# tum-vision/tandem

Measured on AMD Instinct MI355X. Metric: depth-maps/sec @ 640×480×7-view×3-stage; TSDF voxels integrated/sec, higher is better.
Workload: dtype f32; 1 GPU; 640x480 ref+6-src keyframe window, 3-stage cascade (48/32/8 hypotheses), view aggregation, fp32; independent windows, 4 in flight per GPU (one DrMvsnet engine each) x 1 GPU replica(s); trained weights recovered from the reference's exported tandem_512x320 model (same architecture), inputs resident in HBM; height=480, width=640, views=7, parallelism=replicas x1, 4 engines per GPU

## Files before the change

tandem_amd/csrc/dr_mvsnet.hip:

```cpp
#include <atomic>
#include <memory>

#include <dlfcn.h>
#include <rccl/rccl.h>

#include "conv_mfma.h"
#include "mvs_host.h"
#include "mvs_launch.h"
#ifdef DR_PARITY_HOOKS
#include "tail_kernels.h"
#endif
#include "fn_front.h"
#include "fn_head3.h"

namespace dr {

std::string &last_error_slot() {
  thread_local std::string s;
  return s;
}

struct DevTensor {
  float *d = nullptr;
  int D = 0, H = 0, W = 0, C = 0;
  int pad = 0;
  int split = 0;
  size_t n() const { return (size_t)D * (H + 2 * pad) * (W + 2 * pad) * C; }
  float *interior() const { return d + ((size_t)pad * (W + 2 * pad) + pad) * C; }
};

struct Op {
  enum Kind { PREPROCESS, CONV, SKIPUP, PROB, COSTVOL, REGRESS, EDGE, HIST, SCAN, APPLY, BORDERFIX, TAIL, FRONT, HEAD3 } kind;
  const float *p0 = nullptr, *p1 = nullptr, *p3 = nullptr, *p4 = nullptr;
  float *p2 = nullptr;
  int d0 = 0, d1 = 0, d2 = 0;
  std::string name;
  ConvLaunch conv;
#ifdef DR_PARITY_HOOKS
  TailArgs tail{};
#endif
  FrontArgs front{};
  Head3Args head3{};
  PreprocessArgs pre{};
  std::function<ConvLaunch(int)> replan;
  std::string sig;
  int ncand = 0;
  int stage = 0, shift = 0, bits = 0;
  double flops = 0, bytes = 0;
};

struct Rccl {
  void *lib = nullptr;
  decltype(&ncclGetUniqueId) GetUniqueId = nullptr;
  decltype(&ncclCommInitRank) CommInitRank = nullptr;
  decltype(&ncclCommDestroy) CommDestroy = nullptr;
  decltype(&ncclAllReduce) AllReduce = nullptr;
  decltype(&ncclReduce) Reduce = nullptr;
  decltype(&ncclBroadcast) Broadcast = nullptr;
  decltype(&ncclGetErrorString) GetErrorString = nullptr;
  decltype(&ncclCommCount) CommCount = nullptr;
  static Rccl &get() {
    static Rccl r;
    static std::mutex m;
    std::lock_guard<std::mutex> g(m);
    if (!r.lib) {
      if (const char *e = getenv("DR_RCCL_LIB")) r.lib = dlopen(e, RTLD_NOW | RTLD_GLOBAL);
      else
      for (const char *n : {"librccl.so.1", "librccl.so", "/opt/rocm/lib/librccl.so.1"})
        if ((r.lib = dlopen(n, RTLD_NOW | RTLD_GLOBAL))) break;
      if (!r.lib) fail(DR_ERR_UNSUPPORTED, "RCCL not found (librccl.so.1): %s", dlerror());
      r.GetUniqueId = reinterpret_cast<decltype(r.GetUniqueId)>(dlsym(r.lib, "ncclGetUniqueId"));
      r.CommInitRank = reinterpret_cast<decltype(r.CommInitRank)>(dlsym(r.lib, "ncclCommInitRank"));
      r.CommDestroy = reinterpret_cast<decltype(r.CommDestroy)>(dlsym(r.lib, "ncclCommDestroy"));
      r.AllReduce = reinterpret_cast<decltype(r.AllReduce)>(dlsym(r.lib, "ncclAllReduce"));
      r.Reduce = reinterpret_cast<decltype(r.Reduce)>(dlsym(r.lib, "ncclReduce"));
      r.Broadcast = reinterpret_cast<decltype(r.Broadcast)>(dlsym(r.lib, "ncclBroadcast"));
      r.GetErrorString = reinterpret_cast<decltype(r.GetErrorString)>(dlsym(r.lib, "ncclGetErrorString"));
      r.CommCount = reinterpret_cast<decltype(r.CommCount)>(dlsym(r.lib, "ncclCommCount"));
      if (!r.GetUniqueId || !r.CommInitRank || !r.CommDestroy || !r.AllReduce || !r.Reduce || !r.Broadcast || !r.GetErrorString) {
        r.lib = nullptr;
        fail(DR_ERR_UNSUPPORTED, "RCCL: missing symbols in librccl");
      }
    }
    return r;
  }
  void check(ncclResult_t e, const char *what) const {
    if (e != ncclSuccess) fail(DR_ERR_DEVICE, "RCCL %s: %s", what, GetErrorString(e));
  }
};

static const char *conv_kind_name(const ConvLaunch &c) {
  return c.async == 2 ? (c.march.rm ? "rowmarch" : (c.march.wino ? "winomarch" : "march")) : (c.async == 4 ? "wino" : (c.async ? "async" : ""));
}

class MvsEngine {
// ... 240 lines not shown
    DR_HIP(hipSetDevice(device_));
    const DevTensor &t = T(name);
    const size_t logical = (size_t)t.D * t.H * t.W * t.C;
    if (n) *n = logical;
    if (dims) { dims[0] = t.D; dims[1] = t.H; dims[2] = t.W; dims[3] = t.C; }
    if (out) {
      if (logical > n_max) fail(DR_ERR_ARG, "get_tensor(%s): need %zu floats, have %zu", name, logical, n_max);
      DR_HIP(hipStreamSynchronize(stream_));
      check_march();
      if (t.split) {
        const size_t npos = (size_t)t.D * t.H * t.W;
        for (int k = 0; k < t.C / t.split; ++k)
          DR_HIP(hipMemcpy2D(out + (size_t)k * t.split, (size_t)t.C * 4, t.d + (size_t)k * npos * t.split, (size_t)t.split * 4, (size_t)t.split * 4, npos, hipMemcpyDeviceToHost));
      } else if (!t.pad) DR_HIP(hipMemcpy(out, t.d, logical * 4, hipMemcpyDeviceToHost));
      else
        for (int z = 0; z < t.D; ++z)
          DR_HIP(hipMemcpy2D(out + (size_t)z * t.H * t.W * t.C, (size_t)t.W * t.C * 4, t.interior() + (size_t)z * (t.H + 2 * t.pad) * (t.W + 2 * t.pad) * t.C,
                             (size_t)(t.W + 2 * t.pad) * t.C * 4, (size_t)t.W * t.C * 4, t.H, hipMemcpyDeviceToHost));
    }
  }
  void profile(std::string &names, std::vector<float> &ms) {
    std::unique_lock<std::mutex> lk(mu_);
    require_config();
    if (comm_ && shard_nsrc_) fail(DR_ERR_PROTOCOL, "profile(): a view-sharded engine enqueues collectives -- every rank would have to profile in lockstep");
    DR_HIP(hipSetDevice(device_));
    forward(nullptr);
    std::vector<hipEvent_t> ev(ops_.size() + 1);
    for (auto &e : ev) DR_HIP(hipEventCreate(&e));
    forward(&ev);
    DR_HIP(hipStreamSynchronize(stream_));
    check_march();
    names.clear(); ms.clear();
    for (size_t i = 0; i < ops_.size(); ++i) {
      float t = 0;
      DR_HIP(hipEventElapsedTime(&t, ev[i], ev[i + 1]));
      ms.push_back(t);
      const Op &o = ops_[i];
      char kn[64] = "misc";
      if (o.kind == Op::CONV && o.conv.async == 2) snprintf(kn, sizeof kn, "k_conv_m<%d,%d,%d,%d,%d,%d,%d>", o.conv.ci, o.conv.nup, o.conv.ct, o.conv.pt, o.conv.fz, o.conv.ncw, o.conv.march.wino);
      else if (o.kind == Op::CONV && o.conv.async == 4) snprintf(kn, sizeof kn, "k_conv_w<%d,%d,%d>", o.conv.ci, o.conv.ct, o.conv.pt);
      else if (o.kind == Op::CONV && o.conv.async) snprintf(kn, sizeof kn, "k_conv_a<%d,%d,%d>", o.conv.ci, o.conv.ct, o.conv.pt);
      else if (o.kind == Op::CONV && o.conv.bf3) snprintf(kn, sizeof kn, "k_conv_b<%d,%d,%d>", o.conv.ci, o.conv.ct, o.conv.pt);
      else if (o.kind == Op::CONV && o.conv.args.class_loop > 0) snprintf(kn, sizeof kn, "k_conv_c<%d,%d,%d>", o.conv.ci, o.conv.ct, o.conv.pt);
      else if (o.kind == Op::CONV) snprintf(kn, sizeof kn, "k_conv<%d,%d,%d,%d>", o.conv.ci, o.conv.ct, o.conv.pt, o.conv.fz);
      else if (o.kind == Op::COSTVOL) choose_costvol(costvol_shape(cv_[o.stage - 1]), sw_, o.stage).name(kn, sizeof kn);
      else if (o.kind == Op::PROB) choose_prob(prob_shape(pr_[o.stage - 1]), sw_, o.stage).name(kn, sizeof kn);
#ifdef DR_PARITY_HOOKS
      else if (o.kind == Op::TAIL) snprintf(kn, sizeof kn, o.tail.wmf ? "k_tail_m<%d>" : "k_tail<%d>", std::max(3, tail_nout(o.tail.QY, o.tail.QX)));
#endif
      else if (o.kind == Op::REGRESS) snprintf(kn, sizeof kn, "k_regress");
      else if (o.kind == Op::PREPROCESS) snprintf(kn, sizeof kn, "k_preprocess");
      else if (o.kind == Op::FRONT) snprintf(kn, sizeof kn, "k_fn_front");
      else if (o.kind == Op::HEAD3) snprintf(kn, sizeof kn, "k_fn_head3");
      else if (o.kind == Op::SKIPUP) snprintf(kn, sizeof kn, "k_skip_up<%d>", o.stage);
      else if (o.kind == Op::BORDERFIX) snprintf(kn, sizeof kn, "k_out3_border");
      else snprintf(kn, sizeof kn, "k_filter");
      char line[256];
      snprintf(line, sizeof line, "%s\t%s\t%.6e\t%.6e\n", o.name.c_str(), kn, o.flops, o.bytes);
      names += line;
    }
    for (auto &e : ev) (void)hipEventDestroy(e);
  }
  void work(double *flops, double *bytes) {
    std::unique_lock<std::mutex> lk(mu_);
    require_config();
    double f = 0, b = 0;
    for (auto &o : ops_) { f += o.flops; b += o.bytes; }
    if (flops) *flops = f;
    if (bytes) *bytes = b;
  }

 private:
  void check_args(int H, int W, int V, int ref, const uint8_t *const *bgrs, const float *K9, const float *const *c2ws) {
    if (!bgrs || !K9 || !c2ws) fail(DR_ERR_ARG, "CallAsync: null pointer argument");
    const int vmin = shard_nsrc_ ? 1 : 2;
    if (V < vmin || V > kMaxSrc + 1) fail(DR_ERR_ARG, "CallAsync: view_num=%d unsupported (%d..%d)", V, vmin, kMaxSrc + 1);
    if (ref < 0 || ref >= V) fail(DR_ERR_ARG, "CallAsync: ref_index=%d out of range", ref);
    if (H <= 0 || W <= 0 || H % 32 || W % 32) fail(DR_ERR_ARG, "CallAsync: height/width must be positive multiples of 32 (got %dx%d)", H, W);
    for (int i = 0; i < V - 1; ++i) for (int j = i + 1; j < V; ++j)
      if (bgrs[i] == bgrs[j] || c2ws[i] == c2ws[j])
        fail(DR_ERR_ARG, "ERROR: In Call Async passing the same data for index %d and %d", i, j);
  }
  void require_config() { if (!H_) fail(DR_ERR_PROTOCOL, "no window uploaded yet"); }
  void rethrow_worker_error() {
    if (!worker_error_.empty()) { std::string e = worker_error_; worker_error_.clear(); fail(DR_ERR_DEVICE, "%s", e.c_str()); }
  }
  const float *take_result(std::unique_lock<std::mutex> &lk) {
    done_cv_.wait(lk, [&] { return !unprocessed_; });
    rethrow_worker_error();
    if (!has_output_) fail(DR_ERR_PROTOCOL, "Output should be valid. Maybe you called GetResult more than once?");
    has_output_ = false;
    return h_out_[out_cur_];
  }
  static std::atomic<int> &windows_in_flight(int device) {
    static std::atomic<int> n[16];
    return n[device & 15];
  }
  struct InFlight {
    int dev;
    InFlight(int d, bool counted_already) : dev(d) { if (!counted_already) windows_in_flight(dev).fetch_add(1, std::memory_order_relaxed); }
    ~InFlight() { windows_in_flight(dev).fetch_sub(1, std::memory_order_relaxed); }
  };
  void loop() {
    std::unique_lock<std::mutex> lk(mu_);
    while (running_) {
      if (unprocessed_) {
// ... 112 lines not shown
      if (P.launches.size() == 1) {
        o.replan = replan; o.ncand = ncand;
        char sig[160];
        snprintf(sig, sizeof sig, "%d, %d, %d, %d, %d, %d, %d, %d, %d, %d, %d, %d, %d", L.Cin, L.Cout, k3d, kh, kw, L.sd, L.sh, L.sw, L.transposed ? 1 : (L.up2 ? 1 + L.up2 : 0),
                 (int)mode + (fused ? 8 : 0) + (iS ? 16 : 0), iD, iH, iW);
        o.sig = sig;
      }
      o.flops = cl.flops;
      if (idx == 0) o.bytes = 4.0 * ((fused ? in.n() / in.C * fzc.cin + in.n() / 4 : in.n()) + out.n() + add_n);
      if (fused) o.flops += 2.0 * fzc.cin * in.C * (in.n() / in.C);
      ops_.push_back(o);
      ++idx;
    }
  }
  bool lds_fits(size_t bytes) const {
    int optin = 0;
    if (hipDeviceGetAttribute(&optin, hipDeviceAttributeSharedMemPerBlockOptin, device_) != hipSuccess || optin <= 0) {
      (void)hipGetLastError();
      if (hipDeviceGetAttribute(&optin, hipDeviceAttributeMaxSharedMemoryPerBlock, device_) != hipSuccess) { (void)hipGetLastError(); return false; }
    }
    return (size_t)optin >= bytes;
  }
  DevTensor &front_block(const std::string &fn, int V, int H, int W) {
    const HostTensor &wa = blob_.at(fn + "conv0.0.conv.weight"), &wb = blob_.at(fn + "conv0.1.conv.weight");
    const bool shape_ok = wa.dims.size() == 4 && wa.dims[0] == 8 && wa.dims[1] == 3 && wa.dims[2] == 3 && wa.dims[3] == 3 &&
                          wb.dims.size() == 4 && wb.dims[0] == 8 && wb.dims[1] == 8 && wb.dims[2] == 3 && wb.dims[3] == 3;
    const bool fits32 = (double)V * H * W * 32.0 < 2147483648.0 && ((uintptr_t)d_bgr_ & 3) == 0;
    if (!sw_.fn_front || conv_bf3_policy() || !shape_ok || !fits32 || !lds_fits(kFrontLdsBytes)) {
      DevTensor &img = alloc("image", V, H, W, 4);
      { Op o; o.kind = Op::PREPROCESS; o.name = "preprocess"; o.bytes = (double)V * H * W * (3 + 16); o.pre = {d_bgr_, reinterpret_cast<float4 *>(img.d), lut_, (size_t)V * H * W}; ops_.push_back(o); }
      DevTensor &c3a = cbr2("fn.conv0.0", fn + "conv0.0", img, 3, 1, CONV_XPAIR);
      return cbr2("fn.conv0.1", fn + "conv0.1", c3a, 3, 1, CONV_XPAIR);
    }
    DevTensor &c3 = alloc("fn.conv0.1", V, H, W, 8);
    Op o; o.kind = Op::FRONT; o.name = "fn.front";
    FrontArgs &a = o.front;
    a.bgr = d_bgr_; a.lut = lut_; a.out = c3.d;
    a.w1 = reinterpret_cast<const float4 *>(plan_arena_->upload(front_pack(wa.data.data(), 3, 4)));
    a.w2 = reinterpret_cast<const float4 *>(plan_arena_->upload(front_pack(wb.data.data(), 8, 8)));
    auto affine = [&](const std::string &bn) {
      std::vector<float> sc, bi, sb(32);
      fold_bn(blob_, bn, 8, sc, bi);
      for (int r = 0; r < 16; ++r) { sb[r] = sc[r & 7]; sb[16 + r] = bi[r & 7]; }
      return plan_arena_->upload(sb);
    };
    a.sb1 = affine(fn + "conv0.0.bn"); a.sb2 = affine(fn + "conv0.1.bn");
    a.V = V; a.H = H; a.W = W;
    a.tilesY = cdiv(H, kFrontTY); a.tilesX = cdiv(W, kFrontTXP); a.ntiles = V * a.tilesY * a.tilesX;
    o.flops = 2.0 * V * H * W * 9.0 * (4 * 8 + 8 * 8);
    o.bytes = (double)V * H * W * (3 + 32);
    ops_.push_back(o);
    return c3;
  }
  DevTensor &cbr2(const std::string &name, const std::string &p, const DevTensor &in, int k, int s, ConvMode m) {
    return add_conv(name, p + ".conv", p + ".bn", false, true, in, name, 1, k, k, 1, s, s, false, m, nullptr, 0);
  }
  DevTensor &cbr3(const std::string &name, const std::string &p, const DevTensor &in, int sd, int shw, ConvMode m) {
    return add_conv(name, p + ".conv", p + ".bn", false, true, in, name, 3, 3, 3, sd, shw, shw, false, m, nullptr, 0);
  }
  DevTensor &dbr3(const std::string &name, const std::string &p, const DevTensor &in, int sd, const DevTensor &skip) {
    return add_conv(name, p + ".conv", p + ".bn", false, true, in, name, 3, 3, 3, sd, 2, 2, true, CONV_NORMAL, &skip, 1);
  }

  void configure(int H, int W, int V) {
    if (H == H_ && W == W_ && V == V_) return;
    DR_HIP(hipStreamSynchronize(stream_));
    release();
    H_ = W_ = V_ = 0;
    memset(cv_, 0, sizeof cv_);
    memset(rg_, 0, sizeof rg_);
    memset(pr_, 0, sizeof pr_);
    try {
      build_plan(H, W, V);
    } catch (...) {
      release();
      throw;
    }
    H_ = H; W_ = W; V_ = V;
  }
  void build_featurenet(int V, int H, int W) {
    const std::string fn = "feature_net.";
    DevTensor &c3 = front_block(fn, V, H, W);
    DevTensor &c2a = cbr2("fn.conv1.0", fn + "conv1.0", c3, 5, 2, CONV_NORMAL);
    DevTensor &c2b = cbr2("fn.conv1.1", fn + "conv1.1", c2a, 3, 1, CONV_NORMAL);
    DevTensor &c2 = cbr2("fn.conv1.2", fn + "conv1.2", c2b, 3, 1, CONV_NORMAL);
    DevTensor &c1a = cbr2("fn.conv2.0", fn + "conv2.0", c2, 5, 2, CONV_NORMAL);
    DevTensor &c1b = cbr2("fn.conv2.1", fn + "conv2.1", c1a, 3, 1, CONV_NORMAL);
    DevTensor &c1 = cbr2("fn.conv2.2", fn + "conv2.2", c1b, 3, 1, CONV_NORMAL);
    const int fpad = sw_.costvol_v1 ? 0 : 1;
    add_conv("fn.out1", fn + "out.stage1", "", false, false, c1, "feat1", 1, 1, 1, 1, 1, 1, false, CONV_NORMAL, nullptr, 0, nullptr, fpad);
    fork_lo_ = ops_.size();
    DevTensor &i2 = add_skip("fn.skip2", fn + "skip.stage2", c2, "inter2", c1);
    add_conv("fn.out2", fn + "out.stage2", "", false, false, i2, "feat2", 1, 3, 3, 1, 1, 1, false, CONV_NORMAL, nullptr, 0, nullptr, fpad);
    feat2_op_ = ops_.size() - 1;
    const HostTensor &w3 = blob_.at(fn + "skip.stage3.weight");
    const HostTensor &wo3 = blob_.at(fn + "out.stage3.weight");
    if (sw_.out3_folded && !sw_.no_skip_fusion && !sw_.skip_on_conv && w3.dims[0] == 32 && w3.dims[1] == 8 && c3.C == 8 &&
        i2.C == 32 && wo3.dims[0] == 8 && wo3.dims[1] == 32 && i2.H * 2 == c3.H && i2.W * 2 == c3.W) {
      const Out3Fold fold = compose_out3(wo3.data, w3.data, blob_.at(fn + "skip.stage3.bias").data);
      const std::vector<float> &wa = fold.wa, &T = fold.T, &bint = fold.bint;
      DevTensor &f3 = alloc("feat3", c3.D, c3.H, c3.W, 8, fpad);
      if (sw_.fn_head3 && !conv_bf3_policy() && (double)f3.n() * 4.0 < 2147483648.0 && (double)i2.n() * 4.0 < 2147483648.0 && lds_fits(kH3LdsBytes)) {
        Op o; o.kind = Op::HEAD3; o.name = "fn.head3";
        Head3Args &a = o.head3;
        a.c0 = c3.d; a.i2 = i2.d;
        a.wa = reinterpret_cast<const float4 *>(plan_arena_->upload(h3_pack_a(wa.data())));
        a.wb = reinterpret_cast<const float4 *>(plan_arena_->upload(h3_pack_b(wo3.data.data())));
        std::vector<float> b16(16);
        for (int r = 0; r < 16; ++r) b16[r] = bint[r & 7];
        a.bias16 = plan_arena_->upload(b16); a.T = plan_arena_->upload(T);
        a.out = f3.interior(); a.V = c3.D; a.H = c3.H; a.W = c3.W;
        a.out_row = (f3.W + 2 * f3.pad) * 8; a.out_plane = (f3.H + 2 * f3.pad) * a.out_row;
        a.tilesY = cdiv(c3.H, kH3TY); a.tilesX = cdiv(c3.W, kH3TXP); a.ntiles = c3.D * a.tilesY * a.tilesX;
        o.flops = 2.0 * c3.D * c3.H * c3.W * (9.0 * 8 * 8 + 4.0 * 32 * 8);
        o.bytes = 4.0 * (c3.n() + i2.n() + (double)c3.D * c3.H * c3.W * 8);
        ops_.push_back(o);
      } else {
      ConvLayer LA; LA.Cin = 8; LA.Cout = 8; LA.kd = 1; LA.kh = 3; LA.kw = 3; LA.weight = wa.data(); LA.bias = bint; LA.out_pad = fpad;
      emit_conv("fn.out3a", LA, CONV_XPAIR, c3, f3, nullptr, 0, 0);
      for (int py = 0; py < 2; ++py) {
        ConvLayer LB; LB.Cin = 32; LB.Cout = 8; LB.kd = 1; LB.kh = 3; LB.kw = 3; LB.weight = wo3.data.data(); LB.up2 = 1 + py; LB.out_pad = fpad;
        emit_conv(py ? "fn.out3c" : "fn.out3b", LB, CONV_NORMAL, i2, f3, f3.interior(), 1, f3.n() / 2);
      }
      Op o; o.kind = Op::BORDERFIX; o.name = "fn.out3d"; o.p2 = f3.interior(); o.p1 = plan_arena_->upload(T); o.d0 = c3.D; o.d1 = c3.H; o.d2 = c3.W;
      o.stage = fpad; o.bytes = 64.0 * c3.D * (c3.H + c3.W);
      ops_.push_back(o);
      }
    } else
    if (!sw_.no_skip_fusion && !sw_.skip_on_conv && kParityHooks && w3.dims[0] == 32 && w3.dims[1] == 8 && c3.C == 8 && i2.C == 32 &&
        i2.H * 2 == c3.H && i2.W * 2 == c3.W) {
      ConvFuse fz{c3.d, plan_arena_->upload(w3.data), plan_arena_->upload(blob_.at(fn + "skip.stage3.bias").data), i2.d, 8};
      DevTensor virt; virt.D = c3.D; virt.H = c3.H; virt.W = c3.W; virt.C = 32; virt.d = nullptr;
      add_conv("fn.out3", fn + "out.stage3", "", false, false, virt, "feat3", 1, 3, 3, 1, 1, 1, false, CONV_XPAIR, nullptr, 0, &fz, fpad);
    } else {
      DevTensor &i3 = add_skip("fn.skip3", fn + "skip.stage3", c3, "inter3", i2);
      add_conv("fn.out3", fn + "out.stage3", "", false, false, i3, "feat3", 1, 3, 3, 1, 1, 1, false, CONV_XPAIR, nullptr, 0, nullptr, fpad);
    }
    fork_hi_ = ops_.size();
  }

  struct FnOut { size_t op; int stage; size_t offset; };
  struct FcBuffers { float *feat[3] = {nullptr, nullptr, nullptr}; uint8_t *bgr = nullptr; };
  static bool same_instance(const ConvLaunch &a, const ConvLaunch &b) {
    return a.async == b.async && a.ci == b.ci && a.ct == b.ct && a.pt == b.pt && a.fz == b.fz && a.bf3 == b.bf3 && a.nup == b.nup && a.ncw == b.ncw &&
           a.march.wino == b.march.wino && a.march.rm == b.march.rm;
  }
  void build_fn1(int H, int W) {
    fn1_ok_ = false; ops1_.clear(); fcache_.clear(); fc_.clear();
    if (ops_.empty() || ops_[0].kind != Op::FRONT || sw_.costvol_v1 || shard_nsrc_) return;
    const size_t lo = fork_lo_, hi = fork_hi_, f2 = feat2_op_;
    std::vector<Op> batch;
    batch.swap(ops_);
    tprefix_ = "c1.";
    try { build_featurenet(1, H, W); } catch (...) { tprefix_.clear(); ops_.swap(batch); fork_lo_ = lo; fork_hi_ = hi; feat2_op_ = f2; throw; }
    tprefix_.clear();
    ops1_.swap(ops_); ops_.swap(batch);
    fork_lo_ = lo; fork_hi_ = hi; feat2_op_ = f2;
    if (!match_fn1()) { ops1_.clear(); return; }
    const size_t img_bytes = (size_t)H * W * 3;
    fcache_.resize(fcache_cap_); fc_.resize(fcache_cap_);
    for (FcBuffers &e : fcache_) {
      for (int s = 0; s < 3; ++s) {
        const DevTensor &t = T("c1.feat" + std::to_string(s + 1));
        e.feat[s] = dalloc<float>(t.n()); misc_.push_back(e.feat[s]);
        DR_HIP(hipMemset(e.feat[s], 0, t.n() * 4));
      }
      e.bgr = dalloc<uint8_t>(img_bytes + 16); misc_.push_back(e.bgr);
    }
    if (!fc_flag_) { DR_HIP(hipHostMalloc((void **)&fc_flag_, sizeof(int), hipHostMallocDefault)); *fc_flag_ = 0; }
    if (!up_stream_) { DR_HIP(hipStreamCreateWithFlags(&up_stream_, hipStreamNonBlocking)); DR_HIP(hipEventCreateWithFlags(&ev_hits_, hipEventDisableTiming)); }
    fn1_out_.clear();
    for (size_t i = 0; i < ops1_.size(); ++i) {
      Op &o = ops1_[i];
      float *out = o.kind == Op::CONV ? o.conv.args.out : (o.kind == Op::HEAD3 ? o.head3.out : nullptr);
      for (int s = 0; s < 3 && out; ++s) {
        const DevTensor &t = T("c1.feat" + std::to_string(s + 1));
        if (out >= t.d && out < t.d + t.n()) fn1_out_.push_back({i, s, (size_t)(out - t.d)});
      }
    }
    if (fn1_out_.size() != 3) { ops1_.clear(); fcache_.clear(); fc_.clear(); return; }
    fn1_ok_ = true;
  }
  bool match_fn1() {
    for (Op &o : ops1_) {
      const Op *b = nullptr;
      for (size_t i = 0; i < fork_hi_ && i < ops_.size(); ++i) if (ops_[i].name == o.name) b = &ops_[i];
      if (!b || b->kind != o.kind) return false;
      if (o.kind == Op::FRONT || o.kind == Op::HEAD3) continue;
      if (o.kind != Op::CONV) return false;
      if (same_instance(o.conv, b->conv)) continue;
      if (!o.replan) return false;
      bool found = false;
      for (int r = 0; r < o.ncand && !found; ++r) {
        const ConvLaunch c = o.replan(r);
        if (same_instance(c, b->conv)) { o.conv = c; found = true; }
      }
      if (!found) return false;
    }
    return true;
  }
  void plan_cache_use(int H, int W, int V, const uint8_t *const *bgrs, const int *order) {
    fc_.stand_down();
    if (!fn1_ok_ || shard_nsrc_ || comm_ || phase_mode_) return;
    for (int s = 1; s <= 3; ++s)
      if (choose_costvol(costvol_shape(cv_[s - 1]), sw_, s).family != CostVolChoice::V5) return;
    uint64_t keys[kMaxSrc + 1][2];
    for (int v = 0; v < V; ++v) image_key(bgrs[order[v]], (size_t)H * W * 3, H, W, keys[v]);
    fc_.plan(V, keys);
    for (int s = 0; s < 3; ++s)
      for (int v = 0; v < V; ++v)
        if (fc_.fast) cv_[s].vfeat[v] = fcache_[fc_.slot[v]].feat[s];
  }
  void launch_fn_op(const Op &o, hipStream_t st) {
    if (o.kind == Op::CONV) launch_conv(o.conv, st);
    else if (o.kind == Op::FRONT) launch_fn_front(o.front, st);
    else if (o.kind == Op::HEAD3) launch_fn_head3(o.head3, st);
    else fail(DR_ERR_UNSUPPORTED, "feature cache: op kind %d in the single-view plan", (int)o.kind);
  }
  void enqueue_cache_io() {
    const size_t img_bytes = (size_t)H_ * W_ * 3;
    CacheIoArgs io{};
    for (int v = 0; v < V_; ++v) {
      io.img[v] = reinterpret_cast<const uint4 *>(d_bgr_ + v * img_bytes);
      io.entry[v] = reinterpret_cast<uint4 *>(fcache_[fc_.slot[v]].bgr);
    }
    io.miss = fc_.miss; io.flag = fc_flag_dev(); io.n16 = img_bytes / 16;
    launch_cache_io(io, V_, stream_);
  }
  void forward_cached_features() {
    const size_t img_bytes = (size_t)H_ * W_ * 3;
    if (!defer_cache_io_) enqueue_cache_io();
    if (fc_.miss >= 0) {
      const FcBuffers &e = fcache_[fc_.slot[fc_.miss]];
      for (const FnOut &p : fn1_out_) {
        Op &o = ops1_[p.op];
        (o.kind == Op::CONV ? o.conv.args.out : o.head3.out) = e.feat[p.stage] + p.offset;
      }
      for (Op &o : ops1_) {
        if (o.kind == Op::FRONT) o.front.bgr = d_bgr_ + fc_.miss * img_bytes;
        launch_fn_op(o, stream_);
      }
      fc_.set_valid(fc_.slot[fc_.miss]);
    }
  }
  void fill_cache_from_batch() {
    const size_t img_bytes = (size_t)H_ * W_ * 3;
    for (int v = 0; v < V_; ++v) {
      const FcBuffers &e = fcache_[fc_.slot[v]];
      if (fc_.valid(fc_.slot[v])) continue;
      for (int s = 0; s < 3; ++s) {
        const DevTensor &t = T("feat" + std::to_string(s + 1));
        const size_t n1 = t.n() / t.D;
        DR_HIP(hipMemcpyAsync(e.feat[s], t.d + v * n1, n1 * 4, hipMemcpyDeviceToDevice, stream_));
      }
      DR_HIP(hipMemcpyAsync(e.bgr, d_bgr_ + v * img_bytes, img_bytes, hipMemcpyDeviceToDevice, stream_));
      fc_.set_valid(fc_.slot[v]);
    }
  }
  int *fc_flag_dev() { int *d = nullptr; DR_HIP(hipHostGetDevicePointer((void **)&d, fc_flag_, 0)); return d; }
  bool cache_mismatch_recovered() {
    if (!fc_flag_ || !*fc_flag_) return false;
    *fc_flag_ = 0;
    ++fc_.collisions;
    fc_.invalidate_all();
    fc_.fast = false; fc_.fill = false;
    for (int s = 0; s < 3; ++s) set_batch_vfeat(s);
    forward(nullptr);
    DR_HIP(hipStreamSynchronize(stream_));
    return true;
// ... 199 lines not shown
          if (!pinned) { memcpy(h_in_ + v * img_bytes, src, img_bytes); src = h_in_ + v * img_bytes; }
          DR_HIP(hipMemcpyAsync(d_bgr_ + v * img_bytes, src, img_bytes, hipMemcpyHostToDevice, stream_));
        }
      };
      if (!pinned) {
        copier_.run([&] { upload_views(1); });
        try { upload_views(0); } catch (...) { copier_.wait_quiet(); throw; }
        copier_.wait();
      } else {
        upload_views(1);
        upload_views(0);
      }
      if (pinned) {
        if (!ev_h2d_) DR_HIP(hipEventCreateWithFlags(&ev_h2d_, hipEventDisableTiming));
        DR_HIP(hipEventRecord(ev_h2d_, stream_));
        DR_HIP(hipEventSynchronize(ev_h2d_));
      }

    }
  }

  void forward(std::vector<hipEvent_t> *ev, size_t first = 0, size_t last = ~(size_t)0) {
    if ((fc_.fast || fc_.fill) && !(first == 0 && last >= ops_.size())) {
      fc_.fast = fc_.fill = false;
      for (int s = 0; s < 3; ++s) set_batch_vfeat(s);
    }
    const bool cached = fc_.fast;
    const bool alone = windows_in_flight(device_).load(std::memory_order_relaxed) <= 1;
    const bool fork = side_enabled_ && alone && !ev && first == 0 && last >= ops_.size() && fork_lo_ < fork_hi_ && !cached;
    if (cached) forward_cached_features();
    const bool rooted = comm_ && shard_nsrc_ && !phase_mode_ && !sw_.shard_allreduce;
    bool idle_stage = false;
    size_t i = 0;
    for (const Op &o : ops_) {
      if (ev) DR_HIP(hipEventRecord((*ev)[i], stream_));
      ++i;
      if (i - 1 < first || i - 1 >= last) continue;
      if (cached && i - 1 < fork_hi_) continue;
      if (idle_stage && o.kind != Op::REGRESS) continue;
      const bool on_side = fork && i - 1 >= fork_lo_ && i - 1 < fork_hi_;
      if (fork && i - 1 == fork_lo_) { DR_HIP(hipEventRecord(ev_fork_, stream_)); DR_HIP(hipStreamWaitEvent(side_, ev_fork_, 0)); }
      if (fork && o.kind == Op::COSTVOL && o.stage == 2) DR_HIP(hipStreamWaitEvent(stream_, ev_feat2_, 0));
      if (fork && o.kind == Op::COSTVOL && o.stage == 3) DR_HIP(hipStreamWaitEvent(stream_, ev_feat3_, 0));
      const hipStream_t st = on_side ? side_ : stream_;
      switch (o.kind) {
        case Op::PREPROCESS: launch_preprocess(o.pre, st); break;
        case Op::CONV: launch_conv(o.conv, st); break;
        case Op::BORDERFIX: launch_out3_border(o.p2, o.p1, o.d0, o.d1, o.d2, o.stage, st); break;
        case Op::SKIPUP: launch_skip_up(o.p0, o.p1, o.p3, o.p4, o.p2, o.d0, o.d1, o.d2, st); break;
        case Op::PROB: launch_prob(pr_[o.stage - 1], rg_[o.stage - 1], sw_, o.stage, st); break;
        case Op::TAIL: launch_tail_op(o, st); break;
        case Op::FRONT: launch_fn_front(o.front, st); break;
        case Op::HEAD3: launch_fn_head3(o.head3, st); break;
        case Op::COSTVOL: {
          const CostVolArgs &a = cv_[o.stage - 1];
          if (a.V - 1 <= 0) { const DevTensor &vol = T("volume" + std::to_string(o.stage)); DR_HIP(hipMemsetAsync(vol.d, 0, vol.n() * 4, st)); }
          launch_costvol(a, sw_, o.stage, st);
          if (comm_ && shard_nsrc_ && !phase_mode_) {
            const DevTensor &vol = T("volume" + std::to_string(o.stage));
            Rccl &r = Rccl::get();
            if (rooted) {
              r.check(r.Reduce(vol.d, vol.d, vol.n(), ncclFloat, ncclSum, 0, comm_, st), "ncclReduce");
              idle_stage = comm_rank_ != 0;
            } else r.check(r.AllReduce(vol.d, vol.d, vol.n(), ncclFloat, ncclSum, comm_, st), "ncclAllReduce");
          }
          break;
        }
        case Op::REGRESS: {
          const ProbArgs &pr = pr_[o.stage - 1];
          const bool done = pr.x && choose_prob(prob_shape(pr), sw_, o.stage).regresses();
          if (!idle_stage && !done) launch_regress(rg_[o.stage - 1], sw_, st);
          if (rooted) {
            Rccl &c = Rccl::get();
            const DevTensor &dep = T("depth" + std::to_string(o.stage));
            c.check(c.Broadcast(dep.d, dep.d, dep.n(), ncclFloat, 0, comm_, st), "ncclBroadcast");
            if (o.stage == 3) {
              const DevTensor &cf = T("conf3");
              c.check(c.Broadcast(cf.d, cf.d, cf.n(), ncclFloat, 0, comm_, st), "ncclBroadcast");
            }
            idle_stage = false;
          }
          break;
        }
        case Op::EDGE: launch_edge(filt_, filter_rank_, st); break;
        case Op::HIST: launch_hist(filt_, o.stage, o.d0, o.d1, o.shift, o.bits, st); break;
        case Op::SCAN: launch_scan(filt_, o.shift, o.bits, st); break;
        case Op::APPLY: launch_apply(filt_, o.shift, o.bits, st); break;
      }
      if (on_side && i - 1 == feat2_op_) DR_HIP(hipEventRecord(ev_feat2_, side_));
      if (on_side && i - 1 == fork_hi_ - 1) DR_HIP(hipEventRecord(ev_feat3_, side_));
    }
    if (fc_.fill && first == 0 && last >= ops_.size()) fill_cache_from_batch();
    if (ev) DR_HIP(hipEventRecord((*ev)[i], stream_));
    DR_HIP(hipGetLastError());
  }

  void launch_tail_op([[maybe_unused]] const Op &o, [[maybe_unused]] hipStream_t st) {
#ifdef DR_PARITY_HOOKS
    launch_tail(o.tail, st);
#endif
  }
  hipStream_t side_ = nullptr;
  hipEvent_t ev_fork_ = nullptr, ev_feat2_ = nullptr, ev_feat3_ = nullptr;
  bool side_enabled_ = true;
  size_t fork_lo_ = 0, fork_hi_ = 0, feat2_op_ = 0;
  int fcache_cap_ = 0;
// ... 246 lines not shown
```

tandem_amd/csrc/mvs_host.h:

```cpp
#pragma once
#include <algorithm>
#include <cmath>
#include <condition_variable>
#include <functional>
#include <map>
#include <mutex>
#include <thread>

#include "dr_host.h"

namespace dr {

constexpr int kMaxSrc = 7;

struct HostTensor {
  std::vector<int> dims;
  std::vector<float> data;
};
struct BlobMeta {
  int depth_num[3];
  float ratio[3];
  int view_aggregation, base;
};
struct Blob : BlobMeta {
// ... 260 lines not shown
    std::unique_lock<std::mutex> lk(mu_);
    done_.wait(lk, [&] { return !busy_; });
    if (!error_.empty()) { std::string e = error_; error_.clear(); fail(DR_ERR_DEVICE, "%s", e.c_str()); }
  }
  void wait_quiet() {
    std::unique_lock<std::mutex> lk(mu_);
    done_.wait(lk, [&] { return !busy_; });
    error_.clear();
  }

 private:
  void loop() {
    std::unique_lock<std::mutex> lk(mu_);
    for (;;) {
      cv_.wait(lk, [&] { return busy_ || quit_; });
      if (quit_) return;
      std::function<void()> job = std::move(job_);
      lk.unlock();
      std::string err;
      try { job(); } catch (const std::exception &e) { err = e.what(); }
      lk.lock();
      error_ = err;
      busy_ = false;
      done_.notify_all();
    }
  }
  std::mutex mu_;
  std::condition_variable cv_, done_;
  std::function<void()> job_;
  std::string error_;
  bool busy_ = false, quit_ = false;
  std::thread th_;
};

struct MvsSwitches {
  static int num(const char *name, int dflt) { const char *e = getenv(name); return e ? atoi(e) : dflt; }
  static bool on(const char *name) { return getenv(name) != nullptr; }
  static int hnum(const char *name, int dflt) { const char *e = hook_env(name); return e ? atoi(e) : dflt; }
  static bool hon(const char *name) { return hook_env(name) != nullptr; }
  bool side_stream = !on("DR_MVS_NO_SIDE_STREAM");
  int conv_print = num("DR_CONV_PRINT", 0);
  std::string autotune_only = getenv("DR_AUTOTUNE_ONLY") ? getenv("DR_AUTOTUNE_ONLY") : "";
  int cv_dchunk[3] = {num("DR_CV_DCHUNK1", 0), num("DR_CV_DCHUNK2", 0), num("DR_CV_DCHUNK3", 0)};
  int prob_zchunk = num("DR_PROB_ZCHUNK", 0);
  int hist_blocks = std::max(1, num("DR_HIST_BLOCKS", 128));
  int prob_rows = hnum("DR_PROB_ROWS", 0);
  bool costvol_v2 = hon("DR_COSTVOL_V2");
  bool regress_generic = hon("DR_REGRESS_GENERIC");
  bool shard_allreduce = hon("DR_SHARD_ALLREDUCE");
  int tail_fused = hnum("DR_TAIL_FUSED", 0);
  int tail_qy = hnum("DR_TAIL_QY", 0), tail_zchunk = hnum("DR_TAIL_ZCHUNK", 0);
  bool fn_front = hnum("DR_FN_FRONT", 1) != 0;
  bool fn_head3 = hnum("DR_FN_HEAD3", 1) != 0;
  bool filter_fused = hnum("DR_FILTER_FUSED", 1) != 0;
  bool prob_regress = hnum("DR_PROB_REGRESS", 1) != 0;
  bool vol_split = !hon("DR_VOL_NO_SPLIT");
  bool costvol_v1 = hon("DR_COSTVOL_V1");
  bool costvol_v3 = hon("DR_COSTVOL_V3");
  int costvol_cpl = hnum("DR_COSTVOL_CPL", 4) == 8 ? 8 : 4;
  bool prob_v1 = hon("DR_PROB_V1");
  int prob_block = std::max(64, std::min(256, hnum("DR_PROB_BLOCK", 256) / 64 * 64)), prob_xo = hnum("DR_PROB_XO", 1);
  bool prob_launch_order = hon("DR_PROB_LAUNCH_ORDER"), prob_on_conv = hon("DR_PROB_ON_CONV");
  bool skip_on_conv = hon("DR_SKIP_ON_CONV"), no_skip_fusion = hon("DR_NO_SKIP_FUSION");
  bool out3_folded = hnum("DR_OUT3_FOLDED", 1) != 0;
  bool d2h_copy = hook_env("DR_MVS_D2H") && !strcmp(hook_env("DR_MVS_D2H"), "copy");
  int cv5_rows = hnum("DR_CV5_ROWS", 0);
  bool cv5_reuse = hnum("DR_CV5_REUSE", 1) != 0;
  int cv5_abl = hnum("DR_CV5_ABL", 0);
  int cv4_stages = hnum("DR_CV4_STAGES", 0);
  int cv4_sp8 = hnum("DR_CV4_SP8", 0);
};

struct CostVolShape { int V, h, w, D, dchunk, fpad, view_aggregation; };
inline int costvol_dchunk(int stage, int D, int view_aggregation, int fpad, const MvsSwitches &sw) {
  int dchunk = stage == 1 ? 4 : (D >= 16 ? 8 : D);
  if (view_aggregation && fpad && D % 4 == 0 && !sw.costvol_v2 && !sw.costvol_v3 && !sw.cv4_stages) dchunk = 4;
  if (sw.cv_dchunk[stage - 1] > 0) dchunk = std::min(D, sw.cv_dchunk[stage - 1]);
  return dchunk;
}
struct CostVolChoice {
  enum Family { V1, V2, V3, V4, V5 } family;
  int C;
  int a, b, c;
  void name(char *kn, size_t n) const {
    if (family == V4 || family == V5) snprintf(kn, n, family == V4 ? "k_costvol4<%d,%d>" : "k_costvol5<%d,%d>", C, a);
    else snprintf(kn, n, family == V1 ? "k_costvol<%d>" : (family == V2 ? "k_costvol2<%d>" : "k_costvol3<%d>"), C);
  }
};
inline CostVolChoice choose_costvol(const CostVolShape &a, const MvsSwitches &sw, int stage) {
  const int C = 32 >> (stage - 1);
  if (!a.fpad) return {CostVolChoice::V1, C, C >= 16 ? sw.costvol_cpl : 4, 0, 0};
  const bool newer = !sw.costvol_v1 && !sw.costvol_v2 && !sw.costvol_v3 && a.view_aggregation && a.V > 1;
  const int tw = C == 8 ? 16 : 8, th = (1024 / C) / tw, dch = a.D >= 8 ? 8 : 4;
  if (newer && ((sw.cv4_stages >> (stage - 1)) & 1) && a.w % tw == 0 && a.h % th == 0 && a.D % dch == 0) {
    const bool sp8 = dch == 8 && C != 32 && ((sw.cv4_sp8 >> (stage - 1)) & 1);
    return {CostVolChoice::V4, C, dch, sp8 ? 8 : 4, 0};
  }
  if (newer && (a.dchunk == 4 || a.dchunk == 8) && a.D % a.dchunk == 0) {
    const bool rows4 = sw.cv5_rows ? sw.cv5_rows == 4 : true;
    if (!sw.cv5_reuse) return {CostVolChoice::V5, C, a.dchunk, 0, 1};
    return {CostVolChoice::V5, C, a.dchunk, 1, rows4 ? 4 : 1};
  }
  const bool v3 = !sw.costvol_v2 && a.dchunk % 4 == 0 && a.D % 4 == 0;
  return {v3 ? CostVolChoice::V3 : CostVolChoice::V2, C, 0, 0, 0};
}

// ... 35 lines not shown
```

Measured before the change: 591.3 depth-maps/s.

## Fuse paired 3x3 feature-net conv layers into one LDS-resident Winograd kernel

Adds k_fn_mid, which runs two consecutive 3x3 conv+BN+ReLU layers of the feature net in one kernel. The intermediate tile stays in LDS with a halo, and the next input tile is prefetched while the current one is processed. This removes the global write and read of the intermediate activation plus one launch per pair, for the conv1 and conv2 blocks. The default mask DR_FN_MID=1 enables only the first (16-channel) pair. The cost is recomputed halo pixels and a heavy LDS footprint that may limit occupancy, and the kernel only engages when the existing planner picks the matching Winograd layout.

After: 594.2 depth-maps/s (median of 6 runs). No clear change (+0.5%).

```diff
diff --git a/tandem_amd/csrc/dr_mvsnet.hip b/tandem_amd/csrc/dr_mvsnet.hip
--- a/tandem_amd/csrc/dr_mvsnet.hip
+++ b/tandem_amd/csrc/dr_mvsnet.hip
@@ -12,6 +12,7 @@
 #endif
 #include "fn_front.h"
 #include "fn_head3.h"
+#include "fn_mid.h"
 
 namespace dr {
 
@@ -30,7 +31,7 @@
 };
 
 struct Op {
-  enum Kind { PREPROCESS, CONV, SKIPUP, PROB, COSTVOL, REGRESS, EDGE, HIST, SCAN, APPLY, BORDERFIX, TAIL, FRONT, HEAD3 } kind;
+  enum Kind { PREPROCESS, CONV, SKIPUP, PROB, COSTVOL, REGRESS, EDGE, HIST, SCAN, APPLY, BORDERFIX, TAIL, FRONT, HEAD3, MID } kind;
   const float *p0 = nullptr, *p1 = nullptr, *p3 = nullptr, *p4 = nullptr;
   float *p2 = nullptr;
   int d0 = 0, d1 = 0, d2 = 0;
@@ -41,6 +42,7 @@
 #endif
   FrontArgs front{};
   Head3Args head3{};
+  MidArgs mid{};
   PreprocessArgs pre{};
   std::function<ConvLaunch(int)> replan;
   std::string sig;
@@ -387,6 +389,7 @@
       else if (o.kind == Op::PREPROCESS) snprintf(kn, sizeof kn, "k_preprocess");
       else if (o.kind == Op::FRONT) snprintf(kn, sizeof kn, "k_fn_front");
       else if (o.kind == Op::HEAD3) snprintf(kn, sizeof kn, "k_fn_head3");
+      else if (o.kind == Op::MID) snprintf(kn, sizeof kn, "k_fn_mid<%d>", o.stage);
       else if (o.kind == Op::SKIPUP) snprintf(kn, sizeof kn, "k_skip_up<%d>", o.stage);
       else if (o.kind == Op::BORDERFIX) snprintf(kn, sizeof kn, "k_out3_border");
       else snprintf(kn, sizeof kn, "k_filter");
@@ -605,6 +608,43 @@
     ops_.push_back(o);
     return c3;
   }
+  DevTensor &mid_block(const std::string &op, int bit, const std::string &fn, const std::string &la, const std::string &lb, const DevTensor &in) {
+    const int C = in.C;
+    auto two_launches = [&]() -> DevTensor & {
+      DevTensor &t = cbr2("fn." + la, fn + la, in, 3, 1, CONV_NORMAL);
+      return cbr2("fn." + lb, fn + lb, t, 3, 1, CONV_NORMAL);
+    };
+    const HostTensor &wa = blob_.at(fn + la + ".conv.weight"), &wb = blob_.at(fn + lb + ".conv.weight");
+    auto shape_ok = [&](const HostTensor &w, const std::string &l) {
+      return w.dims.size() == 4 && w.dims[0] == C && w.dims[1] == C && w.dims[2] == 3 && w.dims[3] == 3 && blob_.t.count(fn + l + ".bn.weight");
+    };
+    const size_t lds = C == 16 ? MidGeo<16>::kLdsBytes : MidGeo<32>::kLdsBytes;
+    const bool fits32 = (double)in.n() * 4.0 < 2147483648.0;
+    if (!(sw_.fn_mid & bit) || (C != 16 && C != 32) || !shape_ok(wa, la) || !shape_ok(wb, lb) || (in.H & 1) || in.pad || in.split || conv_wino_policy() < 1 ||
+        conv_bf3_policy() || !fits32 || !lds_fits(lds))
+      return two_launches();
+    MidLayerPack pk[2];
+    for (int l = 0; l < 2; ++l) {
+      ConvLayer L;
+      L.Cin = C; L.Cout = C; L.kh = 3; L.kw = 3; L.relu = true; L.weight = (l ? wb : wa).data.data();
+      fold_bn(blob_, fn + (l ? lb : la) + ".bn", C, L.scale, L.bias);
+      pk[l] = mid_pack_layer(L, in.D, in.H, in.W);
+    }
+    if (!pk[0].ok || !pk[1].ok) return two_launches();
+    DevTensor &out = alloc("fn." + lb, in.D, in.H, in.W, C);
+    Op o; o.kind = Op::MID; o.name = op; o.stage = C;
+    MidArgs &a = o.mid;
+    a.in = in.d; a.out = out.d;
+    a.w1 = reinterpret_cast<const float4 *>(plan_arena_->upload(pk[0].w)); a.w2 = reinterpret_cast<const float4 *>(plan_arena_->upload(pk[1].w));
+    a.sb1 = plan_arena_->upload(pk[0].sb); a.sb2 = plan_arena_->upload(pk[1].sb);
+    a.V = in.D; a.H = in.H; a.W = in.W;
+    const int TY = C == 16 ? MidGeo<16>::TY : MidGeo<32>::TY, TX = C == 16 ? MidGeo<16>::TX : MidGeo<32>::TX;
+    a.tilesY = cdiv(in.H, TY); a.tilesX = cdiv(in.W, TX); a.ntiles = in.D * a.tilesY * a.tilesX;
+    o.flops = pk[0].flops + pk[1].flops;
+    o.bytes = 4.0 * (in.n() + out.n() + pk[0].w.size() + pk[1].w.size());
+    ops_.push_back(o);
+    return out;
+  }
   DevTensor &cbr2(const std::string &name, const std::string &p, const DevTensor &in, int k, int s, ConvMode m) {
     return add_conv(name, p + ".conv", p + ".bn", false, true, in, name, 1, k, k, 1, s, s, false, m, nullptr, 0);
   }
@@ -635,11 +675,9 @@
     const std::string fn = "feature_net.";
     DevTensor &c3 = front_block(fn, V, H, W);
     DevTensor &c2a = cbr2("fn.conv1.0", fn + "conv1.0", c3, 5, 2, CONV_NORMAL);
-    DevTensor &c2b = cbr2("fn.conv1.1", fn + "conv1.1", c2a, 3, 1, CONV_NORMAL);
-    DevTensor &c2 = cbr2("fn.conv1.2", fn + "conv1.2", c2b, 3, 1, CONV_NORMAL);
+    DevTensor &c2 = mid_block("fn.mid1", 1, fn, "conv1.1", "conv1.2", c2a);
     DevTensor &c1a = cbr2("fn.conv2.0", fn + "conv2.0", c2, 5, 2, CONV_NORMAL);
-    DevTensor &c1b = cbr2("fn.conv2.1", fn + "conv2.1", c1a, 3, 1, CONV_NORMAL);
-    DevTensor &c1 = cbr2("fn.conv2.2", fn + "conv2.2", c1b, 3, 1, CONV_NORMAL);
+    DevTensor &c1 = mid_block("fn.mid2", 2, fn, "conv2.1", "conv2.2", c1a);
     const int fpad = sw_.costvol_v1 ? 0 : 1;
     add_conv("fn.out1", fn + "out.stage1", "", false, false, c1, "feat1", 1, 1, 1, 1, 1, 1, false, CONV_NORMAL, nullptr, 0, nullptr, fpad);
     fork_lo_ = ops_.size();
@@ -739,7 +777,7 @@
       const Op *b = nullptr;
       for (size_t i = 0; i < fork_hi_ && i < ops_.size(); ++i) if (ops_[i].name == o.name) b = &ops_[i];
       if (!b || b->kind != o.kind) return false;
-      if (o.kind == Op::FRONT || o.kind == Op::HEAD3) continue;
+      if (o.kind == Op::FRONT || o.kind == Op::HEAD3 || o.kind == Op::MID) continue;
       if (o.kind != Op::CONV) return false;
       if (same_instance(o.conv, b->conv)) continue;
       if (!o.replan) return false;
@@ -768,6 +806,7 @@
     if (o.kind == Op::CONV) launch_conv(o.conv, st);
     else if (o.kind == Op::FRONT) launch_fn_front(o.front, st);
     else if (o.kind == Op::HEAD3) launch_fn_head3(o.head3, st);
+    else if (o.kind == Op::MID) launch_fn_mid(o.mid, o.stage, st);
     else fail(DR_ERR_UNSUPPORTED, "feature cache: op kind %d in the single-view plan", (int)o.kind);
   }
   void enqueue_cache_io() {
@@ -1073,6 +1112,7 @@
         case Op::TAIL: launch_tail_op(o, st); break;
         case Op::FRONT: launch_fn_front(o.front, st); break;
         case Op::HEAD3: launch_fn_head3(o.head3, st); break;
+        case Op::MID: launch_fn_mid(o.mid, o.stage, st); break;
         case Op::COSTVOL: {
           const CostVolArgs &a = cv_[o.stage - 1];
           if (a.V - 1 <= 0) { const DevTensor &vol = T("volume" + std::to_string(o.stage)); DR_HIP(hipMemsetAsync(vol.d, 0, vol.n() * 4, st)); }
diff --git a/tandem_amd/csrc/fn_mid.h b/tandem_amd/csrc/fn_mid.h
--- /dev/null
+++ b/tandem_amd/csrc/fn_mid.h
@@ -0,0 +1,283 @@
+#pragma once
+#include <algorithm>
+#include <atomic>
+#include <vector>
+
+#ifndef DR_HD
+#if defined(__HIPCC__)
+#define DR_HD __host__ __device__
+#else
+#define DR_HD
+#endif
+#endif
+
+namespace dr {
+
+constexpr int kMidThreads = 512, kMidWaves = 8;
+constexpr int kMidCIS = 20;
+constexpr int kMidNU = 12;
+
+template <int C>
+struct MidGeo {
+  static_assert(C == 16 || C == 32, "k_fn_mid: 16 or 32 channels");
+  static constexpr int NPL = C / 16, CT = C / 16;
+  static constexpr int TY = C == 16 ? 16 : 4, TX = C == 16 ? 32 : 16;
+  static constexpr int MH = TY + 4, MW = TX + 2;
+  static constexpr int IH = TY + 6, IW = TX + 4;
+  static constexpr int NPI = IH * IW, NPM = MH * MW;
+  static constexpr int NP1 = (MH / 2) * MW, G1 = (NP1 + 15) / 16, PT1 = (G1 + kMidWaves - 1) / kMidWaves;
+  static constexpr int NP2 = (TY / 2) * TX, G2 = NP2 / 16, PT2 = (G2 + kMidWaves - 1) / kMidWaves;
+  static constexpr int PA1 = G1 / kMidWaves, R1 = G1 % kMidWaves, PA2 = G2 / kMidWaves, R2 = G2 % kMidWaves;
+  static constexpr int NF = NPI * NPL * 4;
+  static constexpr int PPT = (NF + kMidThreads - 1) / kMidThreads;
+  static constexpr int WF4 = NPL * kMidNU * CT * 64;
+  static constexpr size_t kLdsBytes = (size_t)NPL * (NPI + NPM) * kMidCIS * 4 + 2 * (size_t)WF4 * 16 + 64;
+  static_assert(TY % 2 == 0 && NP2 % 16 == 0 && PPT <= 32, "tile shape");
+};
+
+struct MidArgs {
+  const float *in;
+  float *out;
+  const float4 *w1, *w2;
+  const float *sb1, *sb2;
+  int V, H, W, tilesY, tilesX, ntiles;
+};
+
+template <int C> DR_HD inline void mid_pos1(int n, int &P, int &mx) { P = n / MidGeo<C>::MW; mx = n - P * MidGeo<C>::MW; }
+template <int C> DR_HD inline int mid_base1(int P, int mx) { return (2 * P * MidGeo<C>::IW + mx) * kMidCIS; }
+template <int C> DR_HD inline void mid_pos2(int n, int &Y, int &ox) { Y = n / MidGeo<C>::TX; ox = n - Y * MidGeo<C>::TX; }
+template <int C> DR_HD inline int mid_base2(int Y, int ox) { return ((2 * Y + 1) * MidGeo<C>::MW + ox) * kMidCIS; }
+template <int C> DR_HD inline void mid_fetch_elem(int n, int &iy, int &ix, int &cc, int &dst) {
+  const int pos = n / (MidGeo<C>::NPL * 4);
+  cc = n - pos * (MidGeo<C>::NPL * 4);
+  iy = pos / MidGeo<C>::IW; ix = pos - iy * MidGeo<C>::IW;
+  dst = (cc >> 2) * MidGeo<C>::NPI * kMidCIS + pos * kMidCIS + (cc & 3) * 4;
+}
+
+struct MidLayerPack {
+  bool ok = false;
+  std::vector<float> w, sb;
+  double flops = 0;
+};
+inline MidLayerPack mid_pack_layer(const ConvLayer &L, int D, int H, int W) {
+  MidLayerPack r;
+  DeviceArena host;
+  host.host_only = true;
+  float in = 0, out = 0;
+  int ncand = 1;
+  for (int rank = 0; rank < ncand && !r.ok; ++rank) {
+    const ConvPlanOut P = plan_conv(L, CONV_NORMAL, &in, D, H, W, L.Cin, &out, nullptr, 0, host, rank);
+    ncand = std::max(1, P.ncand);
+    if (P.launches.size() != 1) continue;
+    const ConvLaunch &c = P.launches[0];
+    const ConvArgs &a = c.args;
+    if (c.async != 4 || c.ci != 16 || a.cls[0].NU != kMidNU || a.npass * 16 != L.Cin || a.ctTot * 16 != L.Cout || a.rows_valid != L.Cout || !a.relu) continue;
+    const float *w = reinterpret_cast<const float *>(a.wpk + a.cls[0].w_base);
+    r.w.assign(w, w + (size_t)a.npass * kMidNU * a.ctTot * 64 * 4);
+    r.sb.assign(a.scale, a.scale + L.Cout);
+    r.sb.insert(r.sb.end(), a.bias, a.bias + L.Cout);
+    r.flops = c.flops;
+    r.ok = true;
+  }
+  return r;
+}
+
+#ifdef __HIPCC__
+template <int C, int PT>
+__device__ inline void mid_round1(const float *tin, float *tmid, const float4 *w1, const int *tapl, int lane, int gi0, const float4 (&sc1)[C / 16],
+                                  const float4 (&bi1)[C / 16], int y0, int x0, int H, int W) {
+  using G = MidGeo<C>;
+  constexpr int CT = G::CT, CIS = kMidCIS;
+  const int j = lane & 15, g = lane >> 4;
+  int b1[PT], P1[PT], mx1[PT];
+  bool ok1[PT];
+#pragma unroll
+  for (int pt = 0; pt < PT; ++pt) {
+    const int n = (gi0 + kMidWaves * pt) * 16 + j;
+    ok1[pt] = n < G::NP1;
+    mid_pos1<C>(ok1[pt] ? n : 0, P1[pt], mx1[pt]);
+    b1[pt] = mid_base1<C>(P1[pt], mx1[pt]) + 4 * g;
+  }
+  floatx4 acc[4][CT][PT];
+#pragma unroll
+  for (int p = 0; p < 4; ++p)
+#pragma unroll
+    for (int ct = 0; ct < CT; ++ct)
+#pragma unroll
+      for (int pt = 0; pt < PT; ++pt) acc[p][ct][pt] = floatx4{0.f, 0.f, 0.f, 0.f};
+#pragma unroll
+  for (int p = 0; p < G::NPL; ++p)
+    conv_w_kloop<CT, PT>(tin + p * G::NPI * CIS, w1 + p * kMidNU * CT * 64, tapl, 1, 3, lane, b1, G::IW * CIS, acc);
+#pragma unroll
+  for (int pt = 0; pt < PT; ++pt) {
+    if (!ok1[pt]) continue;
+    const int gx = x0 - 1 + mx1[pt];
+#pragma unroll
+    for (int ct = 0; ct < CT; ++ct) {
+      const floatx4 m0 = acc[0][ct][pt], m1 = acc[1][ct][pt], m2 = acc[2][ct][pt], m3 = acc[3][ct][pt];
+      const floatx4 o[2] = {(m0 + m1) + m2, (m1 - m2) - m3};
+      const float4 sc = sc1[ct], bi = bi1[ct];
+#pragma unroll
+      for (int r = 0; r < 2; ++r) {
+        const int gy = y0 - 2 + 2 * P1[pt] + r;
+        float4 q;
+        q.x = fmaxf(o[r][0] * sc.x + bi.x, 0.f);
+        q.y = fmaxf(o[r][1] * sc.y + bi.y, 0.f);
+        q.z = fmaxf(o[r][2] * sc.z + bi.z, 0.f);
+        q.w = fmaxf(o[r][3] * sc.w + bi.w, 0.f);
+        if (gy < 0 || gy >= H || gx < 0 || gx >= W) q = make_float4(0.f, 0.f, 0.f, 0.f);
+        *reinterpret_cast<float4 *>(tmid + ct * G::NPM * CIS + ((2 * P1[pt] + r) * G::MW + mx1[pt]) * CIS + 4 * g) = q;
+      }
+    }
+  }
+}
+template <int C, int PT, class F>
+__device__ inline void mid_round2(const float *tmid, float *out, const float4 *w2, const int *tapl, int lane, int gi0, bool active, const float4 (&sc2)[C / 16],
+                                  const float4 (&bi2)[C / 16], int v, int y0, int x0, int H, int W, F between) {
+  using G = MidGeo<C>;
+  constexpr int CT = G::CT, CIS = kMidCIS;
+  const int j = lane & 15, g = lane >> 4;
+  int b2[PT], Y2[PT], ox2[PT];
+#pragma unroll
+  for (int pt = 0; pt < PT; ++pt) {
+    mid_pos2<C>(active ? (gi0 + kMidWaves * pt) * 16 + j : 0, Y2[pt], ox2[pt]);
+    b2[pt] = mid_base2<C>(Y2[pt], ox2[pt]) + 4 * g;
+  }
+  floatx4 acc[4][CT][PT];
+#pragma unroll
+  for (int p = 0; p < 4; ++p)
+#pragma unroll
+    for (int ct = 0; ct < CT; ++ct)
+#pragma unroll
+      for (int pt = 0; pt < PT; ++pt) acc[p][ct][pt] = floatx4{0.f, 0.f, 0.f, 0.f};
+  if (active) {
+#pragma unroll
+    for (int p = 0; p < G::NPL; ++p)
+      conv_w_kloop<CT, PT>(tmid + p * G::NPM * CIS, w2 + p * kMidNU * CT * 64, tapl, 1, 3, lane, b2, G::MW * CIS, acc);
+  }
+  between();
+  if (!active) return;
+#pragma unroll
+  for (int pt = 0; pt < PT; ++pt) {
+    const int gx = x0 + ox2[pt];
+    if (gx >= W) continue;
+#pragma unroll
+    for (int ct = 0; ct < CT; ++ct) {
+      const floatx4 m0 = acc[0][ct][pt], m1 = acc[1][ct][pt], m2 = acc[2][ct][pt], m3 = acc[3][ct][pt];
+      const floatx4 o[2] = {(m0 + m1) + m2, (m1 - m2) - m3};
+      const float4 sc = sc2[ct], bi = bi2[ct];
+#pragma unroll
+      for (int r = 0; r < 2; ++r) {
+        const int gy = y0 + 2 * Y2[pt] + r;
+        if (gy >= H) continue;
+        float4 q;
+        q.x = fmaxf(o[r][0] * sc.x + bi.x, 0.f);
+        q.y = fmaxf(o[r][1] * sc.y + bi.y, 0.f);
+        q.z = fmaxf(o[r][2] * sc.z + bi.z, 0.f);
+        q.w = fmaxf(o[r][3] * sc.w + bi.w, 0.f);
+        *reinterpret_cast<float4 *>(out + (size_t)(unsigned)(((v * H + gy) * W + gx) * C + ct * 16 + 4 * g)) = q;
+      }
+    }
+  }
+}
+
+template <int C>
+__global__ __launch_bounds__(kMidThreads, 2) void k_fn_mid(const MidArgs a) {
+  using G = MidGeo<C>;
+  constexpr int CT = G::CT, CIS = kMidCIS;
+  extern __shared__ float4 lds4[];
+  float *tin = reinterpret_cast<float *>(lds4);
+  float *tmid = tin + G::NPL * G::NPI * CIS;
+  float4 *w1 = reinterpret_cast<float4 *>(tmid + G::NPL * G::NPM * CIS);
+  float4 *w2 = w1 + G::WF4;
+  int *tapl = reinterpret_cast<int *>(w2 + G::WF4);
+  const int tid = threadIdx.x, lane = tid & 63, wave = __builtin_amdgcn_readfirstlane(tid >> 6), g = lane >> 4;
+
+  for (int i = tid; i < G::WF4; i += kMidThreads) { w1[i] = a.w1[i]; w2[i] = a.w2[i]; }
+  if (tid < 3) tapl[tid] = tid * CIS;
+  float4 sc1[CT], bi1[CT], sc2[CT], bi2[CT];
+#pragma unroll
+  for (int ct = 0; ct < CT; ++ct) {
+    sc1[ct] = *reinterpret_cast<const float4 *>(a.sb1 + ct * 16 + 4 * g); bi1[ct] = *reinterpret_cast<const float4 *>(a.sb1 + C + ct * 16 + 4 * g);
+    sc2[ct] = *reinterpret_cast<const float4 *>(a.sb2 + ct * 16 + 4 * g); bi2[ct] = *reinterpret_cast<const float4 *>(a.sb2 + C + ct * 16 + 4 * g);
+    asm volatile("" ::"v"(sc1[ct].x), "v"(sc1[ct].y), "v"(sc1[ct].z), "v"(sc1[ct].w), "v"(bi1[ct].x), "v"(bi1[ct].y), "v"(bi1[ct].z), "v"(bi1[ct].w));
+    asm volatile("" ::"v"(sc2[ct].x), "v"(sc2[ct].y), "v"(sc2[ct].z), "v"(sc2[ct].w), "v"(bi2[ct].x), "v"(bi2[ct].y), "v"(bi2[ct].z), "v"(bi2[ct].w));
+  }
+
+  const int per_xcd = (a.ntiles + 7) >> 3, xcd = blockIdx.x & 7, wi = blockIdx.x >> 3, nw = gridDim.x >> 3;
+  const int t_lo = xcd * per_xcd, t_hi = min(a.ntiles, t_lo + per_xcd);
+  const int my_tiles = t_lo + wi < t_hi ? (t_hi - t_lo - wi + nw - 1) / nw : 0;
+  auto origin = [&](int k, int &v, int &y0, int &x0) {
+    int b = t_lo + wi + k * nw;
+    const int tx = b % a.tilesX;
+    b /= a.tilesX;
+    v = b / a.tilesY; y0 = (b % a.tilesY) * G::TY; x0 = tx * G::TX;
+  };
+  float4 pv[G::PPT];
+  unsigned pin = 0;
+  auto fetch = [&](int k) {
+    int v, y0, x0;
+    origin(k, v, y0, x0);
+    pin = 0;
+#pragma unroll
+    for (int e = 0; e < G::PPT; ++e) {
+      int iy, ix, cc, dst;
+      mid_fetch_elem<C>(e * kMidThreads + tid, iy, ix, cc, dst);
+      const int gy = y0 - 3 + iy, gx = x0 - 2 + ix;
+      const bool in = e * kMidThreads + tid < G::NF && (unsigned)gy < (unsigned)a.H && (unsigned)gx < (unsigned)a.W;
+      const unsigned off = in ? (unsigned)(((v * a.H + gy) * a.W + gx) * C + cc * 4) : 0u;
+      pv[e] = *reinterpret_cast<const float4 *>(a.in + (size_t)off);
+      pin |= in ? 1u << e : 0u;
+    }
+  };
+  auto commit = [&]() {
+#pragma unroll
+    for (int e = 0; e < G::PPT; ++e) {
+      int iy, ix, cc, dst;
+      mid_fetch_elem<C>(e * kMidThreads + tid, iy, ix, cc, dst);
+      if (e * kMidThreads + tid < G::NF) *reinterpret_cast<float4 *>(tin + dst) = (pin >> e) & 1u ? pv[e] : make_float4(0.f, 0.f, 0.f, 0.f);
+    }
+  };
+
+  if (my_tiles > 0) fetch(0);
+  __syncthreads();
+  if (my_tiles > 0) commit();
+  for (int k = 0; k < my_tiles; ++k) {
+    int v, y0, x0;
+    origin(k, v, y0, x0);
+    __syncthreads();
+    if (k + 1 < my_tiles) fetch(k + 1);
+
+    if (G::PA1 > 0) mid_round1<C, (G::PA1 > 0 ? G::PA1 : 1)>(tin, tmid, w1, tapl, lane, wave, sc1, bi1, y0, x0, a.H, a.W);
+    if (wave < G::R1) mid_round1<C, 1>(tin, tmid, w1, tapl, lane, wave + kMidWaves * G::PA1, sc1, bi1, y0, x0, a.H, a.W);
+    __syncthreads();
+
+    auto next_in = [&]() { if (k + 1 < my_tiles) commit(); };
+    auto nothing = []() {};
+    if (G::PA2 > 0 && G::R2 > 0) mid_round2<C, (G::PA2 > 0 ? G::PA2 : 1)>(tmid, a.out, w2, tapl, lane, wave, true, sc2, bi2, v, y0, x0, a.H, a.W, nothing);
+    if (G::PA2 > 0 && G::R2 == 0) mid_round2<C, (G::PA2 > 0 ? G::PA2 : 1)>(tmid, a.out, w2, tapl, lane, wave, true, sc2, bi2, v, y0, x0, a.H, a.W, next_in);
+    if (G::R2 > 0) mid_round2<C, 1>(tmid, a.out, w2, tapl, lane, wave + kMidWaves * G::PA2, wave < G::R2, sc2, bi2, v, y0, x0, a.H, a.W, next_in);
+  }
+}
+
+template <int C>
+inline void launch_fn_mid_inst(const MidArgs &a, hipStream_t st) {
+  static std::atomic<unsigned long long> done{0};
+  int dev = 0;
+  DR_HIP(hipGetDevice(&dev));
+  const unsigned long long bit = 1ull << (dev & 63);
+  if (!(done.load(std::memory_order_acquire) & bit)) {
+    DR_HIP(hipFuncSetAttribute(reinterpret_cast<const void *>(&k_fn_mid<C>), hipFuncAttributeMaxDynamicSharedMemorySize, (int)MidGeo<C>::kLdsBytes));
+    done.fetch_or(bit, std::memory_order_release);
+  }
+  const int want = std::max(1, std::min(a.ntiles, 256));
+  hipLaunchKernelGGL(k_fn_mid<C>, dim3(8 * cdiv(want, 8)), dim3(kMidThreads), MidGeo<C>::kLdsBytes, st, a);
+}
+inline void launch_fn_mid(const MidArgs &a, int C, hipStream_t st) {
+  if (C == 16) launch_fn_mid_inst<16>(a, st);
+  else if (C == 32) launch_fn_mid_inst<32>(a, st);
+  else fail(DR_ERR_UNSUPPORTED, "k_fn_mid: no instance for %d channels", C);
+}
+#endif
+
+}
diff --git a/tandem_amd/csrc/mvs_host.h b/tandem_amd/csrc/mvs_host.h
--- a/tandem_amd/csrc/mvs_host.h
+++ b/tandem_amd/csrc/mvs_host.h
@@ -336,6 +336,7 @@
   int tail_qy = hnum("DR_TAIL_QY", 0), tail_zchunk = hnum("DR_TAIL_ZCHUNK", 0);
   bool fn_front = hnum("DR_FN_FRONT", 1) != 0;
   bool fn_head3 = hnum("DR_FN_HEAD3", 1) != 0;
+  int fn_mid = hnum("DR_FN_MID", 1);
   bool filter_fused = hnum("DR_FILTER_FUSED", 1) != 0;
   bool prob_regress = hnum("DR_PROB_REGRESS", 1) != 0;
   bool vol_split = !hon("DR_VOL_NO_SPLIT");
```
